# ramiyako/vector

Hardware: AMD Instinct MI355X
Metric: Msamples/s c64 through FIR+FFT+xcorr chain; 1/2/4/8 GPU + %HBM roofline (higher is better)
Workload: dtype c64 (fp32)

## Files before the change

vector_amd/csrc/refine.hip:

```cpp
#include "os_common.hpp"

namespace vsig {

#pragma clang fp contract(off)

template <class T> __device__ __forceinline__ double2 ld2(const T* p, long long i);
template <> __device__ __forceinline__ double2 ld2<float2>(const float2* p, long long i) {
  const float2 v = p[i];
  return make_double2((double)v.x, (double)v.y);
}
template <> __device__ __forceinline__ double2 ld2<double2>(const double2* p, long long i) {
  return p[i];
}
__device__ __forceinline__ double2 to_d2(float2 v) { return make_double2((double)v.x, (double)v.y); }
__device__ __forceinline__ double2 to_d2(double2 v) { return v; }

template <class U>
__device__ __forceinline__ void st_agent(U* p, U v) {
  __hip_atomic_store(p, v, __ATOMIC_RELAXED, __HIP_MEMORY_SCOPE_AGENT);
}
template <class U>
__device__ __forceinline__ U ld_agent(const U* p) {
  return __hip_atomic_load(p, __ATOMIC_RELAXED, __HIP_MEMORY_SCOPE_AGENT);
}
__device__ __forceinline__ void stores_done() { __builtin_amdgcn_s_waitcnt(0); }

__device__ __forceinline__ void tap_range(long long i, long long na, long long nv, long long& k0,
                                          long long& k1) {
  const long long lo = (nv - 1) - i;
  const long long hi = na + (nv - 1) - i;
  k0 = lo > 0 ? lo : 0;
  k1 = hi < nv ? hi : nv;
}


struct RefineSlot { double m; long long i; };

constexpr int kNpThreads = 256;
constexpr int kNpGrid = 512;
constexpr int kNpFast = 64;
constexpr int kTile = 2048;
constexpr int kTilePad = 8;
constexpr long long kBlasThreadMin = 10000;
constexpr long long kSparseMax = 4096;

struct RefineGeom {
  long long nout;
  long long F;
  long long na, nv;
  int rev;
  int from_array;
  long long hop;
  int waves, Q, stride;
  int wstep, rsub;
  int cols;
  int nthr;
  long long per_item;
  long long cap;
};

__device__ __forceinline__ long long row_offset(const RefineGeom& g, int w, int q, int l) {
  return (long long)g.wstep * w + l + 64LL * (q % g.rsub) + (long long)g.stride * (q / g.rsub);
}

__device__ __forceinline__ long long item_output(const RefineGeom& g, long long p, int q, int l) {
  const long long b = p / g.waves;
  const int w = (int)(p - b * g.waves);
  const long long ob = b * g.hop;
  const long long rem = g.nout - ob;
  const long long lim = rem < g.hop ? rem : g.hop;
  const long long r = row_offset(g, w, q, l);
  if (r >= lim) return -1;
  const long long raw = ob + r;
  return g.rev ? g.nout - 1 - raw : raw;
}

__device__ __forceinline__ long long entry_output(const RefineGeom& g, const long long* items,
                                                  long long e, long long it0 = -1,
                                                  long long item0 = 0) {
  const long long it = e / g.per_item;
  const int sub = (int)(e - it * g.per_item);
  const long long item = it == it0 ? item0 : ld_agent(items + it);
  if (g.from_array) {
    const long long raw = item * 64 + sub;
    return raw < g.nout ? raw : -1;
  }
  if (g.cols) return item_output(g, item >> 6, sub, (int)(item & 63));
  return item_output(g, item, sub >> 6, sub & 63);
}

__device__ __forceinline__ bool item_span(const RefineGeom& g, long long item, long long& lo,
                                          long long& hi) {
  long long rlo, rhi;
  if (g.from_array) {
    rlo = item * 64;
    if (rlo >= g.nout) return false;
    rhi = rlo + 63 < g.nout - 1 ? rlo + 63 : g.nout - 1;
    lo = rlo;
    hi = rhi;
    return true;
  }
  const long long p = g.cols ? item >> 6 : item;
  const int l = g.cols ? (int)(item & 63) : 0;
  const long long b = p / g.waves;
  const int w = (int)(p - b * g.waves);
  const long long ob = b * g.hop;
  const long long rem = g.nout - ob;
  const long long lim = rem < g.hop ? rem : g.hop;
  if (row_offset(g, w, 0, l) >= lim) return false;
  int qh = (g.cols ? g.cols : g.Q) - 1;
  while (row_offset(g, w, qh, l) >= lim) --qh;
  rlo = ob + row_offset(g, w, 0, l);
  long long top = row_offset(g, w, qh, l) + (g.cols ? 0 : 63);
  if (top >= lim) top = lim - 1;
  rhi = ob + top;
  if (g.rev) {
    lo = g.nout - 1 - rhi;
    hi = g.nout - 1 - rlo;
  } else {
    lo = rlo;
    hi = rhi;
  }
  return true;
}

__device__ __forceinline__ double band_threshold(const PeakPartial* rec, double eps) {
  const double t = rec->max2 * (1.0 - eps);
  return t > 0.0 ? t : 0.0;
}

__global__ __launch_bounds__(256) void refine_select_array(
    const float2* __restrict__ c, long long nout, const PeakPartial* __restrict__ rec, double eps,
    long long* __restrict__ items, RefineKeys* __restrict__ keys) {
  const long long i = (long long)blockIdx.x * 256 + threadIdx.x;
  const double t = band_threshold(rec, eps);
  const bool hit = i < nout && (double)hypotf(c[i].x, c[i].y) >= t;
  const unsigned long long m = __ballot(hit);
  if (hit && (threadIdx.x & 63) == (unsigned)__builtin_ctzll(m)) {
    const long long ch = i >> 6;
    const unsigned long long j = atomicAdd(&keys->count, 1ull);
    items[j] = ch;
    const long long hi = ch * 64 + 63 < nout - 1 ? ch * 64 + 63 : nout - 1;
    atomicMax(&keys->lo_inv, ~(unsigned long long)(ch * 64));
    atomicMax(&keys->hi_p1, (unsigned long long)(hi + 1));
  }
}
// ... 677 lines not shown
      else __builtin_amdgcn_s_sleep(127);
    }
    if (timed_out) watchdog_fired(f);
    skeys[0] = timed_out ? 0 : ld_agent(&f.keys->count);
    skeys[1] = ld_agent(&f.keys->lo_inv);
    skeys[2] = ld_agent(&f.keys->hi_p1);
    sitem0 = it0 < f.maxitems ? ld_agent(f.items + it0) : 0;
    stores_done();
    atomicAdd(&fc->seen, 1ull);
  }
  __syncthreads();
  long long nact;
  const bool last = numpy_pass<T>(a, v, f.g, f.items, f.keys, slots, cv, nullptr, 0, 0, f.rec,
                                  skeys[0], skeys[1], skeys[2], vb, kNpGrid, nact,
                                  (unsigned long long)it0 < skeys[0] ? it0 : -1, sitem0);
  if (tid == 0 && (last || (nact == 0 && vb == 0))) {
    const unsigned long long w0 = wall_clock64();
    while (__hip_atomic_load(&fc->seen, __ATOMIC_RELAXED, __HIP_MEMORY_SCOPE_AGENT) < (unsigned long long)kNpGrid) {
      if (wall_clock64() - w0 > f.wd_ticks) {
        watchdog_fired(f);
        break;
      }
      __builtin_amdgcn_s_sleep(20);
    }
    if (ld_agent(&f.keys->fault)) poison_record(f.rec);
    __hip_atomic_store(&fc->seen, 0ull, __ATOMIC_RELAXED, __HIP_MEMORY_SCOPE_AGENT);
    __hip_atomic_store(&fc->flag, 0ull, __ATOMIC_RELAXED, __HIP_MEMORY_SCOPE_AGENT);
    __hip_atomic_store(&fc->ticket, 0ull, __ATOMIC_RELAXED, __HIP_MEMORY_SCOPE_AGENT);
  }
}

static RefineGeom make_geom(const RefineArgs& r) {
  RefineGeom g{r.nout, r.F, r.na, r.nv, r.rev, r.from_array, r.hop, r.waves, r.Q, r.stride,
               r.wstep, r.rsub, r.cols, r.blas_threads > 1 ? r.blas_threads : 1, 0, r.cap};
  g.per_item = r.from_array ? 64 : r.cols ? r.cols : (long long)r.Q * 64;
  return g;
}

static long long max_items(const RefineArgs& r) {
  if (r.from_array) return (r.nout + 63) / 64;
  return r.cols ? r.nparts * 64 : r.nparts;
}

size_t refine_scratch_bytes(const RefineArgs& r) {
  return sizeof(RefineKeys) + (size_t)max_items(r) * 8 + kNpGrid * sizeof(RefineSlot);
}

static hipError_t launch_numpy(const RefineArgs& r, const RefineGeom& g, const long long* items,
                               RefineKeys* keys, RefineSlot* slots, double* vals, long long vlo,
                               long long vhi, hipStream_t st) {
  auto go = [&](auto tag) {
    using T = decltype(tag);
    hipLaunchKernelGGL(refine_numpy<T>, dim3(kNpGrid), dim3(kNpThreads), 0, st,
                       static_cast<const T*>(r.a), static_cast<const T*>(r.v), g, items, keys,
                       slots, static_cast<double2*>(r.out128), vals, vlo, vhi, r.rec);
  };
  if (r.c128) go(double2{});
  else go(float2{});
  return hipGetLastError();
}

hipError_t launch_refine(const RefineArgs& r, hipStream_t st) {
  if (r.cols && (r.from_array || r.cols > 64)) return hipErrorInvalidValue;
  char* base = static_cast<char*>(r.scratch);
  RefineKeys* keys = reinterpret_cast<RefineKeys*>(base);
  long long* items = reinterpret_cast<long long*>(base + sizeof(RefineKeys));
  RefineSlot* slots = reinterpret_cast<RefineSlot*>(items + max_items(r));
// ... 76 lines not shown
```

vector_amd/csrc/vsig_api.hip:

```cpp
#include <cmath>
#include <cstddef>
#include <cstdio>
#include <cstdlib>
#include <cstring>
#include <map>
#include <memory>
#include <string>
#include <vector>

#include "../../include/vsig.h"
#include "dtype.hpp"

using vsig::PeakPartial;
using vsig::dtype_bytes;
using vsig::dtype_ok;
static_assert(VSIG_DTYPE_C128 == vsig::VSIG_C128 && VSIG_DTYPE_C64 == vsig::VSIG_C64 &&
              VSIG_DTYPE_F64 == vsig::VSIG_F64 && VSIG_DTYPE_F32 == vsig::VSIG_F32, "VSIG_DTYPE_*");

struct TimingRec {
  std::vector<std::pair<hipEvent_t, hipEvent_t>> ev;
};

constexpr int kClockSlots = 32;

// ... 80 lines not shown
  int refine_async = 0;
  struct RefineAsync {
    hipStream_t stream = nullptr;
    hipEvent_t ev_corr = nullptr, ev_ref = nullptr;
    bool pending = false;
    bool joined = false;
    hipStream_t joined_on = nullptr;
  } ra;
  bool clock = false;
  DevBuf clkbuf;
  std::map<std::string, int> clkslot;
};

constexpr int kFirPartTaps = 8192;
struct vsig_fir {
  vsig_ctx* ctx;
  int ntaps, decim, M;
  long long hop;
  DevBuf Hs;
  DevBuf G;
  std::vector<vsig_fir*> parts;
  DevBuf z;
  ~vsig_fir() {
    (void)hipStreamSynchronize(ctx->stream);
    for (vsig_fir* p : parts) delete p;
  }
};

struct vsig_xcorr {
  vsig_ctx* ctx;
  long long L = 0;
  int M = 0;
  std::vector<DevBuf> Ps;
  DevBuf tmpl;
  DevBuf cbuf;
  explicit vsig_xcorr(vsig_ctx* c) : ctx(c) {}
  ~vsig_xcorr() { (void)hipStreamSynchronize(ctx->stream); }
};

constexpr long long kBankMaxL = 4096;
constexpr int kBankMaxK = 4096;
struct vsig_xcorr_bank {
  vsig_ctx* ctx;
  int K = 0;
  long long L = 0;
  int M = 0;
  DevBuf Ps;
  explicit vsig_xcorr_bank(vsig_ctx* c) : ctx(c) {}
  ~vsig_xcorr_bank() { (void)hipStreamSynchronize(ctx->stream); }
};

namespace {

int fail(vsig_ctx* c, int code, const std::string& msg) {
  if (c) c->err = msg;
  return code;
}

void join_refine(vsig_ctx* c) {
  vsig_ctx::RefineAsync& ra = c->ra;
  if (!ra.pending) return;
  if (ra.joined && ra.joined_on == c->stream) return;
  (void)hipStreamWaitEvent(c->stream, ra.ev_ref, 0);
  ra.joined = true;
  ra.joined_on = c->stream;
}
// ... 163 lines not shown

int clear_refine_fault(vsig_ctx* c, unsigned long long fault = 0) {
  char* keys = c->rscratch.as<char>();
  HIPCHK(c, hipMemsetAsync(keys, 0, sizeof(vsig::RefineKeys), c->stream));
  if (fault)
    HIPCHK(c, hipMemcpyAsync(keys + offsetof(vsig::RefineKeys, fault), &fault, sizeof(fault),
                             hipMemcpyHostToDevice, c->stream));
  if (c->parts())
    HIPCHK(c, hipMemsetAsync(c->counters(), 0, vsig::kCounterRecs * sizeof(PeakPartial), c->stream));
  HIPCHK(c, hipStreamSynchronize(c->stream));
  return VSIG_OK;
}

bool corr_span(int mode, long long na, long long nv, long long* F, long long* nout) {
  const long long nmin = na < nv ? na : nv, nmax = na < nv ? nv : na;
  if (mode == VSIG_MODE_FULL) { *F = 0; *nout = na + nv - 1; }
  else if (mode == VSIG_MODE_VALID) { *F = nmin - 1; *nout = nmax - nmin + 1; }
  else if (mode == VSIG_MODE_SAME) { *F = na >= nv ? nmin - 1 - nmin / 2 : nmin / 2; *nout = nmax; }
  else return false;
  return true;
}

bool is_complex_dtype(int dtype) { return dtype == VSIG_DTYPE_C64 || dtype == VSIG_DTYPE_C128; }

struct RefineOperands {
  const void* a; long long na;
  const void* v; long long nv;
  int c128;
  long long F;
};

int run_refine(vsig_ctx* c, const RefineOperands& op, long long nout, int M, long long hop,
               long long nparts, int rev, const float2* c64, PeakPartial* rec, void* out128,
               bool fused = false, const unsigned* lkeys = nullptr, bool async = false) {
  c->refine_ran = false;
  if (!c->refine) return fused ? fail(c, VSIG_E_INVALID, "refine: fused finalize with refine off")
                             : VSIG_OK;
  vsig::RefineArgs r{};
  r.a = op.a; r.na = op.na; r.v = op.v; r.nv = op.nv; r.c128 = op.c128;
  r.nout = nout; r.F = op.F; r.rev = rev;
  if (c64) {
    r.from_array = 1; r.c64 = c64; r.Q = 1; r.stride = 0; r.waves = 1; r.hop = 64;
    r.wstep = 64; r.rsub = 1;
  } else {
    int waves, Q, stride, plan, wstep, rsub;
    if (vsig::xcorr_geom(M, &waves, &Q, &stride, &plan, &wstep, &rsub) != hipSuccess)
      return fail(c, VSIG_E_INVALID, "refine: no correlator geometry for M");
    r.parts = c->parts(); r.nparts = nparts; r.hop = hop;
    r.waves = waves; r.Q = Q; r.stride = stride; r.wstep = wstep; r.rsub = rsub;
    if (fused) {
      r.finalize = 1;
      r.tmp = c->finalize_tmp();
      r.done = reinterpret_cast<unsigned long long*>(c->counters());
    }
    if (lkeys) {
      r.cols = Q; r.lkeys = lkeys; r.Q = 1;
    }
  }
  r.eps = c->refine_eps_ppm * 1e-6;
  r.blas_threads = c->blas_threads;
  r.cap = c->refine_cap;
  r.wd_ticks = (unsigned long long)c->refine_wd_us * 100ull;
  const size_t need = vsig::refine_scratch_bytes(r);
  const bool fresh = need > c->rscratch.bytes();
  unsigned long long pending_fault = 0;
  if (fresh && c->rscratch.data()) {
    vsig::RefineKeys keys;
    int rc = read_refine_keys(c, &keys);
    if (rc) return rc;
    pending_fault = keys.fault;
  }
  int rc = c->rscratch.reserve(c, need);
  if (rc) return rc;
  if (pending_fault) {
    if ((rc = clear_refine_fault(c, pending_fault))) return rc;
  } else if (fresh) {
    HIPCHK(c, hipMemsetAsync(c->rscratch.data(), 0, sizeof(vsig::RefineKeys), c->stream));
  }
  r.scratch = c->rscratch.data();
  r.rec = rec;
  r.out128 = out128;
  if (async && c->refine_async) {
// ... 682 lines not shown

int vsig_fir_c64(vsig_ctx* c, const void* x, int64_t n, const float* taps, int32_t ntaps,
                 int32_t decim, void* y, int64_t ny) {
  if (!c || !x || !taps || !y) return fail(c, VSIG_E_INVALID, "null pointer");
  if (ntaps < 1) return fail(c, VSIG_E_INVALID, "ntaps must be >= 1");
  std::vector<float2> tc(ntaps);
  for (int i = 0; i < ntaps; ++i) tc[i] = make_float2(taps[i], 0.f);
  vsig_fir* f = nullptr;
  int rc = vsig_fir_create(c, tc.data(), ntaps, decim, &f);
  if (rc) return rc;
  const std::unique_ptr<vsig_fir> owner(f);
  const size_t bx = (size_t)n * 8, by = (size_t)ny * 8;
  if ((rc = stage_in(c, 0, x, bx)) || (rc = c->stage[1].reserve(c, by)) ||
      (rc = vsig_fir_exec_dev(f, c->stage[0].data(), n, c->stage[1].data(), ny)) ||
      (rc = stage_out(c, y, c->stage[1], by)))
    return rc;
  HIPCHK(c, hipStreamSynchronize(c->stream));
  return VSIG_OK;
}

static int xcorr_build(vsig_ctx* c, const float2* td, long long L, vsig_xcorr* x) {
  constexpr long long B = 8192;
  x->L = L;
  x->M = os_size_xcorr(L) ? os_size_xcorr(L) : 16384;
  const long long Bc = x->M == 32768 ? 16384 : B;
  for (long long p = 0; p * Bc < L || p == 0; ++p) {
    const long long Lp = L <= Bc ? L : ((L - p * Bc) < B ? (L - p * Bc) : B);
    DevBuf P;
    const int rc = make_spectrum(c, td + p * B, (int)Lp, x->M, &P);
    if (rc) return rc;
    x->Ps.push_back(std::move(P));
    if (L <= Bc) break;
  }
  return VSIG_OK;
}

static int xcorr_run(vsig_xcorr* x, const float2* s, long long n, long long off, long long nout,
                     int store_mode, float2* cout, vsig_peak_t* peak_dev,
                     const RefineOperands* op, void* out128, bool async = false) {
  vsig_ctx* c = x->ctx;
  PeakPartial* rec = peak_record(c, peak_dev);
  if (x->Ps.size() == 1 && x->L <= (x->M == 32768 ? 16384 : 8192)) {
    long long hop = (long long)x->M - x->L + 1;
    if (x->M == 16384 && hop > 1) hop &= ~1LL;
    const long long nblocks = (nout + hop - 1) / hop;
    int waves, Q, stride, plan, wstep, rsub;
    if (vsig::xcorr_geom(x->M, &waves, &Q, &stride, &plan, &wstep, &rsub) != hipSuccess)
      return fail(c, VSIG_E_UNSUPPORTED, "correlator block size");
    const long long nparts = nblocks * waves;
    int rc = ensure_partials(c, nparts);
    if (rc) return rc;
    const bool fused = op && c->refine && !(store_mode & 8);
    unsigned* lk = nullptr;
    if (fused && Q <= 64 && vsig::xcorr_lane_keys(x->M) == Q) {
      if ((rc = c->lkeys.reserve(c, (size_t)nparts * 64 * sizeof(unsigned)))) return rc;
      lk = c->lkeys.as<unsigned>();
    }
    const float2* tw;
    const float2* wt = nullptr;
    if ((rc = get_twiddles(c, plan, &tw))) return rc;
    if (x->M >= 16384 && (rc = get_half_tw(c, x->M, x->M == 16384 ? 512 : 1024, &wt))) return rc;
    {
      Timed t(c, "xcorr");
      HIPCHK(c, vsig::launch_xcorr_os(x->M, s, n, x->Ps[0].as<float2>(), off, nout, hop, cout, store_mode,
                                      c->parts(), tw, wt, c->stream, lk));
    }
    if (!fused) {
      if ((rc = finalize_peak(c, nparts, 1, peak_dev))) return rc;
      if (!op) return VSIG_OK;
    }
    if (out128 && cout) HIPCHK(c, vsig::launch_convert_c(1, cout, nout, out128, c->stream));
    return run_refine(c, *op, nout, x->M, hop, nparts, (store_mode & 4) ? 1 : 0, nullptr, rec, out128,
                      fused, lk, async && peak_dev != nullptr);
  }
  constexpr long long B = 8192;
  constexpr int M = 16384;
  float2* cbuf = cout;
  int rc;
  if (!cbuf) {
    if ((rc = x->cbuf.reserve(c, (size_t)nout * sizeof(float2)))) return rc;
    cbuf = x->cbuf.as<float2>();
  }
  const float2 *tw, *wt;
  int waves, Q, stride, plan, wstep, rsub;
  if (vsig::xcorr_geom(M, &waves, &Q, &stride, &plan, &wstep, &rsub) != hipSuccess)
    return fail(c, VSIG_E_UNSUPPORTED, "correlator block size");
  if ((rc = get_twiddles(c, plan, &tw)) || (rc = get_half_tw(c, M, 512, &wt))) return rc;
  {
    Timed t(c, "xcorr");
    for (size_t p = 0; p < x->Ps.size(); ++p) {
      const long long Lp = (x->L - (long long)p * B) < B ? (x->L - (long long)p * B) : B;
      const int mode = (store_mode & 4 ? 2 | 4 : 1) | (p ? 8 : 0);
      HIPCHK(c, vsig::launch_xcorr_os(M, s, n, x->Ps[p].as<float2>(), off - (long long)p * B, nout,
                                      (long long)M - Lp + 1, cbuf, mode, nullptr, tw, wt,
                                      c->stream));
    }
    if ((rc = vsig_peak_dev(c, VSIG_DTYPE_C64, cbuf, nout, peak_dev))) return rc;
  }
  if (!op) return VSIG_OK;
  if (out128 && cout) HIPCHK(c, vsig::launch_convert_c(1, cout, nout, out128, c->stream));
  return run_refine(c, *op, nout, M, 0, 0, 0, cbuf, rec, out128);
}

int vsig_xcorr_create(vsig_ctx* c, const void* tmpl, int64_t L, vsig_xcorr** out) {
  if (!c || !tmpl || !out) return fail(c, VSIG_E_INVALID, "null pointer");
  *out = nullptr;
  if (L < 1) return fail(c, VSIG_E_INVALID, "template length must be >= 1");
  std::unique_ptr<vsig_xcorr> x(new vsig_xcorr(c));
  hipError_t e = x->tmpl.alloc((size_t)L * sizeof(float2));
  if (e == hipSuccess)
    e = hipMemcpyAsync(x->tmpl.data(), tmpl, (size_t)L * sizeof(float2), hipMemcpyHostToDevice, c->stream);
  if (e != hipSuccess)
    return fail(c, e == hipErrorOutOfMemory ? VSIG_E_NOMEM : VSIG_E_HIP, hipGetErrorString(e));
  const int rc = xcorr_build(c, x->tmpl.as<float2>(), L, x.get());
  (void)hipStreamSynchronize(c->stream);
  if (rc) return rc;
  *out = x.release();
  return VSIG_OK;
}

// ... 780 lines not shown
```

vector_amd/csrc/vsig_kernels.h:

```cpp
#pragma once
#include <hip/hip_runtime.h>

namespace vsig {

__device__ __forceinline__ long long xcd_remap(long long b, long long nb) {
  const long long q = nb >> 3, r = nb & 7;
  const long long x = b & 7, i = b >> 3;
  return x * q + (x < r ? x : r) + i;
}

struct ClockStamp {
  unsigned long long t0 = 0, r0 = 0;
  bool on;
  __device__ __forceinline__ ClockStamp(unsigned long long* sink, unsigned long long blk)
      : on(sink != nullptr && (blk & 63) == 0) {
    if (on) {
      t0 = __builtin_amdgcn_s_memtime();
      r0 = __builtin_amdgcn_s_memrealtime();
      __builtin_amdgcn_s_waitcnt(0xC07F);
    }
  }
  __device__ __forceinline__ void done(unsigned long long* sink) const {
    if (on && threadIdx.x < 2) {
      const unsigned long long t1 = __builtin_amdgcn_s_memtime();
// ... 54 lines not shown

hipError_t launch_psd(int N, const float2* x, long long stride, const float* win, int nperseg,
                      long long hop, float scale, float* out, long long nframes, int shift,
                      const float2* tw, hipStream_t st);
int psd_plan_threads(int N);
hipError_t launch_spectrum_prep(int N, const float2* u, int len, float gain, float2* S,
                                const float2* tw, hipStream_t st);
struct PsdRec { double sum; float mx, mn; };
struct PsdTracesPlan { long long blocks, step, fpb; };
constexpr int kPsdFoldRows = 8;
bool psd_traces_in_lds(long long N);
PsdTracesPlan psd_traces_plan(long long N, long long nframes);
int psd_traces_table(int N, bool* two_level);
hipError_t launch_psd_traces(int N, const float2* x, long long stride, const float* win, int nperseg,
                             long long hop, float scale, long long nframes, int shift, const float2* tw,
                             PsdRec* rows, hipStream_t st);
hipError_t launch_psd_traces_fold(const float* sxx, long long nb, long long N, int first, PsdRec* rows,
                                  hipStream_t st);
hipError_t launch_psd_traces_merge(const PsdRec* rows, long long nrows, long long N, long long nframes,
                                   double* mean, float* mx, float* mn, hipStream_t st);
hipError_t launch_fir_dec(int decim, const float2* x, long long n, long long g0, const float2* Hs,
                          int lo2, long long hop, float2* y, const float2* tw, const float2* twd,
                          hipStream_t st, const MixArgs* mix = nullptr);
hipError_t launch_fir_poly_gtable(const float2* Hs, float2* G, hipStream_t st);
hipError_t launch_fir_poly(const float2* x, long long n, long long g0, const float2* G, int lo2,
                           long long hop, float2* y, const float2* tw, const float2* twd,
                           hipStream_t st, const MixArgs* mix = nullptr);
hipError_t launch_fir_os(int M, const float2* x, long long n, long long g0, const float2* Hs,
                         int ntaps, long long hop, int decim, float2* y, const float2* tw,
                         hipStream_t st, const MixArgs* mix = nullptr);
hipError_t launch_xcorr_os(int M, const float2* s, long long n, const float2* Ps, long long off,
                           long long nout, long long hop, float2* c, int store_mode,
                           PeakPartial* partials, const float2* tw, const float2* wt,
                           hipStream_t st, unsigned* lkeys = nullptr);
int xcorr_lane_keys(int M);
hipError_t xcorr_geom(int M, int* waves, int* Q, int* stride, int* plan, int* wstep, int* rsub);
hipError_t xcorr_bank_geom(int M, long long nblocks, int* waves, long long* grid);
hipError_t launch_xcorr_bank(int M, const float2* s, long long n, const float2* Ps, int K,
                             long long off, long long nout, long long hop, float2* c,
                             PeakPartial* partials, const float2* tw, hipStream_t st);
hipError_t launch_bank_finalize(const PeakPartial* parts, int K, long long nparts, PeakPartial* out,
                                hipStream_t st);
#ifdef VSIG_TUNING
hipError_t launch_fft_bench(int key, float2* io, int frames, int iters, const float2* tw, int twl,
                            hipStream_t st);
hipError_t launch_copy_probe(const float2* x, long long n, float2* y, int variant, int grid,
                             hipStream_t st);
#endif
hipError_t launch_peak_reduce(int dtype, const void* a, long long n, PeakPartial* partials,
                              int nparts, hipStream_t st);
hipError_t launch_peak_first_nan(int dtype, const void* a, long long n, PeakPartial* rec, hipStream_t st);
constexpr int kFinalizeTmp = 1024;
constexpr int kCounterRecs = 4;
hipError_t launch_partial_finalize(const PeakPartial* parts, long long nparts, int sqrt_max,
                                   PeakPartial* out, PeakPartial* tmp, hipStream_t st);

struct RefineArgs {
  const void* a; long long na;
  const void* v; long long nv;
  int c128;
  long long nout, F;
  int rev;
  int from_array;
  const float2* c64;
  const PeakPartial* parts;
  long long nparts, hop;
  int waves, Q, stride;
  int wstep, rsub;
  double eps;
  int blas_threads;
  int cols;
  const unsigned* lkeys;
  int finalize;
  PeakPartial* tmp;
  unsigned long long* done;
  long long cap;
  void* scratch;
  PeakPartial* rec;
  void* out128;
  unsigned long long wd_ticks;
};
struct RefineKeys {
  unsigned long long count;
  unsigned long long lo_inv;
  unsigned long long hi_p1;
  unsigned long long status;
  unsigned long long done;
  unsigned long long fault;
  unsigned long long pad[2];
};
constexpr size_t kRefineKeysBytes = 64;
static_assert(sizeof(RefineKeys) == kRefineKeysBytes, "the items follow the keys at +64 B");
size_t refine_scratch_bytes(const RefineArgs& r);
hipError_t launch_refine(const RefineArgs& r, hipStream_t st);
size_t refine_values_scratch_bytes();
hipError_t launch_refine_values(const RefineArgs& r, long long lo, long long hi, double* vals,
                                hipStream_t st);
size_t np_stats_scratch_bytes(long long n);
hipError_t launch_np_stats(int dtype, const void* a, long long n, double* out, void* scratch,
                           hipStream_t st);
constexpr int kRegionBlocks = 2048;
// ... 119 lines not shown
```

vector_amd/csrc/xcorr.hip:

```cpp
#include "xcorr_epilogue.hpp"

namespace vsig {

template <class P>
__global__ __launch_bounds__(P::TF) void xcorr_os_kernel(
    const float2* __restrict__ s, long long n, const float2* __restrict__ Ps, long long off,
    long long nout, long long hop, float2* __restrict__ c, int store_mode,
    PeakPartial* __restrict__ partials, long long nblocks, const float2* __restrict__ tw) {
  static_assert(P::R[0] == P::RL, "overlap-save needs a palindromic plan");
  __shared__ __attribute__((aligned(16))) float2 lds[lds_size<P>()];
  const int t = threadIdx.x;
  long long b = blockIdx.x;
  if (b >= nblocks) return;
  float2 wa[nanch_total<P>()];
  load_anchors<P>(wa, tw, t);
  float2 v[P::E];
  load_segment<P>(v, s, b * hop - off, n, t);
  for (; b < nblocks; b += gridDim.x) {
    fft_frame_anch<P>(v, lds, wa, t);
#pragma unroll
    for (int e = 0; e < P::E; ++e) v[e] = cmul(cconj(v[e]), Ps[out_index<P>(t, e)]);
    float2 nv[P::E];
    const long long nb = b + gridDim.x;
    if (nb < nblocks) load_segment<P>(nv, s, nb * hop - off, n, t);
// ... 5 lines not shown
}

using PlanX32k = Plan16384w;
using PlanX16k = Plan8192c;
constexpr int kPlanKey16k = -8192;

template <class P, int M>
constexpr int half_root(int e) {
  return ((e / P::R[0]) * P::TF + (e % P::R[0]) * (P::N / P::R[0])) / (M / 64);
}

template <class P>
__device__ __forceinline__ void load_halves(float2* a, float2* d, const float2* __restrict__ x,
                                            long long s0, long long n, int t) {
  constexpr int H = P::N;
  const float2* base = x + s0;
  if (s0 >= 0 && s0 + 2 * H <= n) {
    const auto rs = make_rsrc(base, 2u * H * (unsigned)sizeof(float2));
    const unsigned v0 = (unsigned)in_index<P>(t, 0) * (unsigned)sizeof(float2);
    static_for<0, P::E>([&](auto ei) {
      constexpr int e = decltype(ei)::value;
      a[e] = buf_load2(rs, v0, in_off<P>(e) * (int)sizeof(float2));
      d[e] = buf_load2(rs, v0, (in_off<P>(e) + H) * (int)sizeof(float2));
    });
  } else {
#pragma unroll
    for (int e = 0; e < P::E; ++e) {
      const int i = in_index<P>(t, e);
      const long long x0 = s0 + i, x1 = x0 + H;
      a[e] = (x0 >= 0 && x0 < n) ? base[i] : make_float2(0.f, 0.f);
      d[e] = (x1 >= 0 && x1 < n) ? base[i + H] : make_float2(0.f, 0.f);
    }
  }
}

template <class P>
struct KeyedRank {
  static constexpr int c(int e) { return (e / P::RL) * P::TF + (e % P::RL) * (P::N / P::RL); }
  static constexpr int rank(int e) {
    int r = 0;
    for (int q = 0; q < P::E; ++q) r += c(q) < c(e);
    return r;
  }
  static constexpr int kStep = P::TF < P::N / P::RL ? P::TF : P::N / P::RL;
  static constexpr bool check() {
    if (mapl_of<P>::value == kMapIlv || 2 * P::E > 64 || P::N != kStep * P::E) return false;
    for (int e = 0; e < P::E; ++e)
      if (c(e) != kStep * rank(e)) return false;
    return true;
  }
  static constexpr bool ok = check();
};

template <class P, int DV = -1>
__device__ __forceinline__ void xcorr_half_epilogue(const float2* a, const float2* d, long long b,
                                                    long long hop, long long nout,
                                                    float2* __restrict__ c, int store_mode,
                                                    PeakPartial* partials, unsigned* lkeys, int t) {
  constexpr int H = P::N;
  const long long ob = b * hop;
  const long long rem = nout - ob;
  const int lim = rem < hop ? (int)rem : (int)hop;
  const bool rev = store_mode & 4;
  const bool accum = store_mode & 8;
  const int smode = store_mode & 3;
  if (smode == 1) {
// ... 77 lines not shown
    return;
  }
  float m = -1.f, s1 = 0.f, s2 = 0.f;
  int mi = 0;
  auto acc = [&](float2 v, int i) {
    const bool ok = i < lim;
    const float a2r = v.x * v.x + v.y * v.y;
    const float a2 = ok ? a2r : -1.f;
    const bool take = (a2 > m) | (rev & (a2 == m) & ok);
    m = take ? a2 : m;
    mi = take ? i : mi;
    s1 += ok ? __builtin_amdgcn_sqrtf(a2r) : 0.f;
    s2 += ok ? a2r : 0.f;
  };
  if (!rev && lim > H) {
#pragma unroll
    for (int e = 0; e < P::E; ++e) {
      const float a2 = a[e].x * a[e].x + a[e].y * a[e].y;
      const bool take = a2 > m;
      m = take ? a2 : m;
      mi = take ? out_index<P>(t, e) : mi;
      s1 += __builtin_amdgcn_sqrtf(a2);
      s2 += a2;
    }
  } else {
#pragma unroll
    for (int e = 0; e < P::E; ++e) acc(a[e], out_index<P>(t, e));
  }
#pragma unroll
  for (int e = 0; e < P::E; ++e) acc(d[e], out_index<P>(t, e) + H);
  wave_partial_f(m, mi, s1, s2, rev, ob, nout, partials + b * (P::TF / 64) + (t >> 6));
}

template <class P>
constexpr int xcorr_waves_per_eu() { return P::E <= 16 ? 4 : P::TF >= 512 ? 1 : 2; }

constexpr int kSegPfDist = 64;

template <class P, int DV = -1>
__global__ __launch_bounds__(P::TF, xcorr_waves_per_eu<P>()) void xcorr_half_kernel(
    const float2* __restrict__ s, long long n, const float4* __restrict__ Ps2, long long off,
    long long nout, long long hop, float2* __restrict__ c, int store_mode,
    PeakPartial* __restrict__ partials, long long nblocks, const float2* __restrict__ tw,
    const float2* __restrict__ wt, unsigned* __restrict__ lkeys, unsigned long long* clk) {
  static_assert(P::R[0] == P::RL, "overlap-save needs a palindromic plan");
  static_assert(map0_of<P>::value != kMapIlv, "one split twiddle per thread");
  constexpr int M = 2 * P::N;
  static_assert(P::TF % (M / 64) == 0 && (P::N / P::R[0]) % (M / 64) == 0,
                "per-element split twiddles must be 64th roots of unity");
  __shared__ __attribute__((aligned(16))) float2 lds[lds_size<P>()];
  const int t = threadIdx.x;
  const ClockStamp cs(clk, blockIdx.x);
  float2 wa[nanch_total<P>()];
  load_anchors<P>(wa, tw, t);
  float2 wx[twx_total<P>()];
  load_twx<P>(wx, tw, t);
  const long long b = xcd_remap(blockIdx.x, gridDim.x);
  if (b >= nblocks) return;
  auto fft2 = [&](float2* x, float2* y) {
    launder_anchors<P>(wa);
    fft_pair<P>(x, y, lds, TwAnchorsX{wa, wx}, t);
  };
  const float2 w = wt[in_index<P>(t, 0)];
  float2 a[P::E], d[P::E];
  load_halves<P>(a, d, s, b * hop - off, n, t);
  constexpr int kPfLines = 2 * P::N * 8 / 128 / P::TF;
  float pfv[kPfLines];
#pragma unroll
  for (int k = 0; k < kPfLines; ++k) pfv[k] = 0.f;
  static_for<0, P::E>([&](auto ei) {
    constexpr int e = decltype(ei)::value;
    const float2 x0 = a[e], x1 = d[e];
    a[e] = cadd(x0, x1);
    d[e] = twc<half_root<P, M>(e), 64>(cmul(csub(x0, x1), w));
  });
  fft2(a, d);
  {
    const auto rp = make_rsrc(Ps2, (unsigned)P::N * (unsigned)sizeof(float4));
    const unsigned v0 = (unsigned)out_index<P>(t, 0) * (unsigned)sizeof(float4);
    static_for<0, P::E>([&](auto ei) {
      constexpr int e = decltype(ei)::value;
      const float4 p = buf_load4(rp, v0, out_off<P>(e) * (int)sizeof(float4));
      a[e] = cmul(cconj(a[e]), make_float2(p.x, p.y));
      d[e] = cmul(cconj(d[e]), make_float2(p.z, p.w));
    });
  }
  fft2(a, d);
  static_for<0, P::E>([&](auto ei) {
    constexpr int e = decltype(ei)::value;
    const float2 o = twc<half_root<P, M>(e), 64>(cmul(d[e], w));
    const float2 ev = a[e];
    a[e] = cadd(ev, o);
    d[e] = csub(ev, o);
  });
  {
    const long long bn = b + kSegPfDist;
    const long long s0 = bn * hop - off;
    if (bn < nblocks && s0 >= 0 && s0 + 2 * P::N <= n) {
      const float* q = reinterpret_cast<const float*>(s + s0);
#pragma unroll
      for (int k = 0; k < kPfLines; ++k) pfv[k] = q[(t + k * P::TF) * 32];
    }
  }
  xcorr_half_epilogue<P, DV>(a, d, b, hop, nout, c, store_mode, partials, lkeys, t);
#pragma unroll
  for (int k = 0; k < kPfLines; ++k)
    asm volatile("" ::"v"(pfv[k]));
  cs.done(clk);
}

hipError_t launch_xcorr_os(int M, const float2* s, long long n, const float2* Ps, long long off,
                           long long nout, long long hop, float2* c, int store_mode,
                           PeakPartial* partials, const float2* tw, const float2* wt,
                           hipStream_t st, unsigned* lkeys) {
  if (nout <= 0) return hipSuccess;
  if (lkeys && !xcorr_lane_keys(M)) return hipErrorInvalidValue;
  const long long nblocks = (nout + hop - 1) / hop;
  if (M == 16384) {
    using KR = KeyedRank<PlanX16k>;
    constexpr int kDv = PlanX16k::E / 2;
    const long long cut = hop - PlanX16k::N;
    const bool dv = KR::ok && KR::kStep == PlanX16k::TF && cut == (long long)kDv * KR::kStep;
    if (dv) {
      hipLaunchKernelGGL((xcorr_half_kernel<PlanX16k, kDv>), dim3((unsigned)nblocks),
                         dim3(PlanX16k::TF), 0, st, s, n, reinterpret_cast<const float4*>(Ps), off, nout,
                         hop, c, store_mode, partials, nblocks, tw, wt, lkeys, g_clock_sink);
      return hipGetLastError();
    }
    hipLaunchKernelGGL(xcorr_half_kernel<PlanX16k>, dim3((unsigned)nblocks), dim3(PlanX16k::TF), 0,
                       st, s, n, reinterpret_cast<const float4*>(Ps), off, nout, hop, c, store_mode,
                       partials, nblocks, tw, wt, lkeys, g_clock_sink);
    return hipGetLastError();
  }
  if (M == 32768) {
    hipLaunchKernelGGL(xcorr_half_kernel<PlanX32k>, dim3((unsigned)nblocks), dim3(PlanX32k::TF), 0,
                       st, s, n, reinterpret_cast<const float4*>(Ps), off, nout, hop, c, store_mode,
                       partials, nblocks, tw, wt, lkeys, g_clock_sink);
    return hipGetLastError();
  }
  auto run = [&](auto plan) {
    using PL = decltype(plan);
    auto k = xcorr_os_kernel<PL>;
    const long long grid = persistent_grid(k, PL::TF, nblocks);
    hipLaunchKernelGGL(k, dim3((unsigned)grid), dim3(PL::TF), 0, st, s, n, Ps, off, nout, hop, c,
                       store_mode, partials, nblocks, tw);
  };
  if (M == 4096) run(Plan4096{});
  else if (M == 8192) run(Plan8192{});
  else return hipErrorInvalidValue;
  return hipGetLastError();
}

template <class P>
constexpr int lane_key_rows() {
  return KeyedRank<P>::ok && KeyedRank<P>::kStep == P::TF && 2 * P::E <= 64 ? 2 * P::E : 0;
}
int xcorr_lane_keys(int M) {
  if (M == 16384) return lane_key_rows<PlanX16k>();
  if (M == 32768) return lane_key_rows<PlanX32k>();
  return 0;
}

hipError_t xcorr_geom(int M, int* waves, int* Q, int* stride, int* plan, int* wstep, int* rsub) {
  *wstep = 64;
  *rsub = 1;
  if (M == 32768) { *waves = PlanX32k::TF / 64; *Q = 2 * PlanX32k::E; *stride = PlanX32k::TF; *plan = -16384; }
  else if (M == 16384) {
    *waves = PlanX16k::TF / 64; *Q = 2 * PlanX16k::E; *stride = PlanX16k::TF; *plan = kPlanKey16k;
  }
  else if (M == 8192) { *waves = Plan8192::TF / 64; *Q = Plan8192::E; *stride = Plan8192::TF; *plan = 8192; }
  else if (M == 4096) { *waves = Plan4096::TF / 64; *Q = Plan4096::E; *stride = Plan4096::TF; *plan = 4096; }
  else return hipErrorInvalidValue;
  return hipSuccess;
}

}
```

Measured before the change: 313,600.

## Add even/odd parity-split path for the 16k half-size correlator

Adds a parity variant of the M=16384 half-length correlator. It loads even/odd samples as one float4 and uses a precomputed sum/difference spectrum table (SD) with a folded twiddle. This removes the pre-FFT and post-FFT butterfly/twiddle passes, moving that work into the pointwise multiply with fused complex MACs. Output indexing, peak keys and refine geometry get new lane/row steps so the interleaved layout still maps to the right output positions. The path runs only when the input pointer and offset are parity-aligned, and it costs an extra table buffer plus a new kernel variant.

After: 319,500, median of 6. 1.02x the previous value.

```diff
diff --git a/vector_amd/csrc/refine.hip b/vector_amd/csrc/refine.hip
--- a/vector_amd/csrc/refine.hip
+++ b/vector_amd/csrc/refine.hip
@@ -53,6 +53,7 @@
   long long hop;
   int waves, Q, stride;
   int wstep, rsub;
+  int lstep, rstep;
   int cols;
   int nthr;
   long long per_item;
@@ -60,7 +61,8 @@
 };
 
 __device__ __forceinline__ long long row_offset(const RefineGeom& g, int w, int q, int l) {
-  return (long long)g.wstep * w + l + 64LL * (q % g.rsub) + (long long)g.stride * (q / g.rsub);
+  return (long long)g.wstep * w + (long long)g.lstep * l + (long long)g.rstep * (q % g.rsub) +
+         (long long)g.stride * (q / g.rsub);
 }
 
 __device__ __forceinline__ long long item_output(const RefineGeom& g, long long p, int q, int l) {
@@ -111,7 +113,7 @@
   int qh = (g.cols ? g.cols : g.Q) - 1;
   while (row_offset(g, w, qh, l) >= lim) --qh;
   rlo = ob + row_offset(g, w, 0, l);
-  long long top = row_offset(g, w, qh, l) + (g.cols ? 0 : 63);
+  long long top = g.cols ? row_offset(g, w, qh, l) : row_offset(g, w, qh, 63);
   if (top >= lim) top = lim - 1;
   rhi = ob + top;
   if (g.rev) {
@@ -855,7 +857,8 @@
 
 static RefineGeom make_geom(const RefineArgs& r) {
   RefineGeom g{r.nout, r.F, r.na, r.nv, r.rev, r.from_array, r.hop, r.waves, r.Q, r.stride,
-               r.wstep, r.rsub, r.cols, r.blas_threads > 1 ? r.blas_threads : 1, 0, r.cap};
+               r.wstep, r.rsub, r.lstep ? r.lstep : 1, r.rstep ? r.rstep : 64, r.cols,
+               r.blas_threads > 1 ? r.blas_threads : 1, 0, r.cap};
   g.per_item = r.from_array ? 64 : r.cols ? r.cols : (long long)r.Q * 64;
   return g;
 }
diff --git a/vector_amd/csrc/vsig_api.hip b/vector_amd/csrc/vsig_api.hip
--- a/vector_amd/csrc/vsig_api.hip
+++ b/vector_amd/csrc/vsig_api.hip
@@ -136,6 +136,7 @@
   long long L = 0;
   int M = 0;
   std::vector<DevBuf> Ps;
+  DevBuf SD;
   DevBuf tmpl;
   DevBuf cbuf;
   explicit vsig_xcorr(vsig_ctx* c) : ctx(c) {}
@@ -365,7 +366,8 @@
 
 int run_refine(vsig_ctx* c, const RefineOperands& op, long long nout, int M, long long hop,
                long long nparts, int rev, const float2* c64, PeakPartial* rec, void* out128,
-               bool fused = false, const unsigned* lkeys = nullptr, bool async = false) {
+               bool fused = false, const unsigned* lkeys = nullptr, bool async = false,
+               bool parity = false) {
   c->refine_ran = false;
   if (!c->refine) return fused ? fail(c, VSIG_E_INVALID, "refine: fused finalize with refine off")
                              : VSIG_OK;
@@ -376,11 +378,13 @@
     r.from_array = 1; r.c64 = c64; r.Q = 1; r.stride = 0; r.waves = 1; r.hop = 64;
     r.wstep = 64; r.rsub = 1;
   } else {
-    int waves, Q, stride, plan, wstep, rsub;
-    if (vsig::xcorr_geom(M, &waves, &Q, &stride, &plan, &wstep, &rsub) != hipSuccess)
+    vsig::XcorrGeom g;
+    if (vsig::xcorr_geom(M, parity, &g) != hipSuccess)
       return fail(c, VSIG_E_INVALID, "refine: no correlator geometry for M");
+    const int Q = g.Q;
     r.parts = c->parts(); r.nparts = nparts; r.hop = hop;
-    r.waves = waves; r.Q = Q; r.stride = stride; r.wstep = wstep; r.rsub = rsub;
+    r.waves = g.waves; r.Q = g.Q; r.stride = g.stride; r.wstep = g.wstep; r.rsub = g.rsub;
+    r.lstep = g.lstep; r.rstep = g.rstep;
     if (fused) {
       r.finalize = 1;
       r.tmp = c->finalize_tmp();
@@ -1129,6 +1133,10 @@
     x->Ps.push_back(std::move(P));
     if (L <= Bc) break;
   }
+  if (x->M == 16384 && x->Ps.size() == 1) {
+    HIPCHK(c, x->SD.alloc((size_t)(x->M / 2) * sizeof(float4)));
+    HIPCHK(c, vsig::launch_xcorr_parity_table(x->M, x->Ps[0].as<float2>(), x->SD.as<float4>(), c->stream));
+  }
   return VSIG_OK;
 }
 
@@ -1141,9 +1149,11 @@
     long long hop = (long long)x->M - x->L + 1;
     if (x->M == 16384 && hop > 1) hop &= ~1LL;
     const long long nblocks = (nout + hop - 1) / hop;
-    int waves, Q, stride, plan, wstep, rsub;
-    if (vsig::xcorr_geom(x->M, &waves, &Q, &stride, &plan, &wstep, &rsub) != hipSuccess)
+    const bool parity = x->M == 16384 && x->SD.data() && !(hop & 1) && vsig::xcorr_parity_aligned(s, off);
+    vsig::XcorrGeom g;
+    if (vsig::xcorr_geom(x->M, parity, &g) != hipSuccess)
       return fail(c, VSIG_E_UNSUPPORTED, "correlator block size");
+    const int waves = g.waves, Q = g.Q, plan = g.plan;
     const long long nparts = nblocks * waves;
     int rc = ensure_partials(c, nparts);
     if (rc) return rc;
@@ -1160,7 +1170,8 @@
     {
       Timed t(c, "xcorr");
       HIPCHK(c, vsig::launch_xcorr_os(x->M, s, n, x->Ps[0].as<float2>(), off, nout, hop, cout, store_mode,
-                                      c->parts(), tw, wt, c->stream, lk));
+                                      c->parts(), tw, wt, c->stream, lk,
+                                      parity ? x->SD.as<float4>() : nullptr));
     }
     if (!fused) {
       if ((rc = finalize_peak(c, nparts, 1, peak_dev))) return rc;
@@ -1168,7 +1179,7 @@
     }
     if (out128 && cout) HIPCHK(c, vsig::launch_convert_c(1, cout, nout, out128, c->stream));
     return run_refine(c, *op, nout, x->M, hop, nparts, (store_mode & 4) ? 1 : 0, nullptr, rec, out128,
-                      fused, lk, async && peak_dev != nullptr);
+                      fused, lk, async && peak_dev != nullptr, parity);
   }
   constexpr long long B = 8192;
   constexpr int M = 16384;
@@ -1179,10 +1190,10 @@
     cbuf = x->cbuf.as<float2>();
   }
   const float2 *tw, *wt;
-  int waves, Q, stride, plan, wstep, rsub;
-  if (vsig::xcorr_geom(M, &waves, &Q, &stride, &plan, &wstep, &rsub) != hipSuccess)
+  vsig::XcorrGeom g;
+  if (vsig::xcorr_geom(M, false, &g) != hipSuccess)
     return fail(c, VSIG_E_UNSUPPORTED, "correlator block size");
-  if ((rc = get_twiddles(c, plan, &tw)) || (rc = get_half_tw(c, M, 512, &wt))) return rc;
+  if ((rc = get_twiddles(c, g.plan, &tw)) || (rc = get_half_tw(c, M, 512, &wt))) return rc;
   {
     Timed t(c, "xcorr");
     for (size_t p = 0; p < x->Ps.size(); ++p) {
diff --git a/vector_amd/csrc/vsig_kernels.h b/vector_amd/csrc/vsig_kernels.h
--- a/vector_amd/csrc/vsig_kernels.h
+++ b/vector_amd/csrc/vsig_kernels.h
@@ -110,9 +110,12 @@
 hipError_t launch_xcorr_os(int M, const float2* s, long long n, const float2* Ps, long long off,
                            long long nout, long long hop, float2* c, int store_mode,
                            PeakPartial* partials, const float2* tw, const float2* wt,
-                           hipStream_t st, unsigned* lkeys = nullptr);
+                           hipStream_t st, unsigned* lkeys = nullptr, const float4* SD = nullptr);
+hipError_t launch_xcorr_parity_table(int M, const float2* Ps, float4* SD, hipStream_t st);
+bool xcorr_parity_aligned(const float2* s, long long off);
 int xcorr_lane_keys(int M);
-hipError_t xcorr_geom(int M, int* waves, int* Q, int* stride, int* plan, int* wstep, int* rsub);
+struct XcorrGeom { int waves, Q, stride, plan, wstep, rsub, lstep, rstep; };
+hipError_t xcorr_geom(int M, bool parity, XcorrGeom* g);
 hipError_t xcorr_bank_geom(int M, long long nblocks, int* waves, long long* grid);
 hipError_t launch_xcorr_bank(int M, const float2* s, long long n, const float2* Ps, int K,
                              long long off, long long nout, long long hop, float2* c,
@@ -145,6 +148,7 @@
   long long nparts, hop;
   int waves, Q, stride;
   int wstep, rsub;
+  int lstep, rstep;
   double eps;
   int blas_threads;
   int cols;
diff --git a/vector_amd/csrc/xcorr.hip b/vector_amd/csrc/xcorr.hip
--- a/vector_amd/csrc/xcorr.hip
+++ b/vector_amd/csrc/xcorr.hip
@@ -61,6 +61,47 @@
       d[e] = (x1 >= 0 && x1 < n) ? base[i + H] : make_float2(0.f, 0.f);
     }
   }
+}
+
+template <class P>
+__device__ __forceinline__ void load_parity(float2* a, float2* d, const float2* __restrict__ x,
+                                            long long s0, long long n, int t) {
+  constexpr int H = P::N;
+  const float2* base = x + s0;
+  if (s0 >= 0 && s0 + 2 * H <= n) {
+    const auto rs = make_rsrc(base, 2u * H * (unsigned)sizeof(float2));
+    const unsigned v0 = (unsigned)in_index<P>(t, 0) * (unsigned)sizeof(float4);
+    static_for<0, P::E>([&](auto ei) {
+      constexpr int e = decltype(ei)::value;
+      const float4 q = buf_load4(rs, v0, in_off<P>(e) * (int)sizeof(float4));
+      a[e] = make_float2(q.x, q.y);
+      d[e] = make_float2(q.z, q.w);
+    });
+  } else {
+#pragma unroll
+    for (int e = 0; e < P::E; ++e) {
+      const int i = 2 * in_index<P>(t, e);
+      const long long x0 = s0 + i, x1 = x0 + 1;
+      a[e] = (x0 >= 0 && x0 < n) ? base[i] : make_float2(0.f, 0.f);
+      d[e] = (x1 >= 0 && x1 < n) ? base[i + 1] : make_float2(0.f, 0.f);
+    }
+  }
+}
+
+template <class P>
+constexpr int parity_root(int e) { return out_off<P>(e) / (P::N / 64); }
+
+__device__ __forceinline__ float2 cmac(float2 a, float2 b, float2 acc) {
+  const f2v av = tov(a), bv = tov(b);
+  return cmul_fin(a, b, av * bv.xx + tov(acc));
+}
+__device__ __forceinline__ float2 cmsub(float2 a, float2 b, float2 acc) {
+  const f2v av = tov(a), bv = tov(b);
+  const f2v t = tov(acc) - av * bv.xx;
+  f2v r;
+  asm("v_pk_fma_f32 %0, %1, %2, %3 op_sel:[1,1,0] op_sel_hi:[0,1,1] neg_hi:[1,0,0]"
+      : "=v"(r) : "v"(av), "v"(bv), "v"(t));
+  return fromv(r);
 }
 
 template <class P>
@@ -204,12 +245,96 @@
   wave_partial_f(m, mi, s1, s2, rev, ob, nout, partials + b * (P::TF / 64) + (t >> 6));
 }
 
+template <class P, int DV = -1>
+__device__ __forceinline__ void xcorr_parity_epilogue(const float2* a, const float2* d,
+                                                      long long b, long long hop, long long nout,
+                                                      float2* __restrict__ c, int store_mode,
+                                                      PeakPartial* partials, unsigned* lkeys,
+                                                      int t) {
+  using KR = KeyedRank<P>;
+  static_assert(KR::ok && KR::kStep == P::TF, "the parity split keys by 2 rank + parity");
+  const long long ob = b * hop;
+  const long long rem = nout - ob;
+  const int lim = rem < hop ? (int)rem : (int)hop;
+  const bool rev = store_mode & 4;
+  const bool accum = store_mode & 8;
+  const int smode = store_mode & 3;
+  if (smode == 1) {
+#pragma unroll
+    for (int e = 0; e < P::E; ++e) {
+      const int i = 2 * out_index<P>(t, e);
+      if (i < lim) put_c(c + ob + (unsigned)i, cconj(a[e]), accum);
+      if (i + 1 < lim) put_c(c + ob + (unsigned)(i + 1), cconj(d[e]), accum);
+    }
+  } else if (smode == 2) {
+#pragma unroll
+    for (int e = 0; e < P::E; ++e) {
+      const int i = 2 * out_index<P>(t, e);
+      if (i < lim) put_c(c + (nout - 1 - ob) - i, a[e], accum);
+      if (i + 1 < lim) put_c(c + (nout - 1 - ob) - (i + 1), d[e], accum);
+    }
+  }
+  if (!partials) return;
+  auto keyed = [&](auto revc) {
+    constexpr bool kRev = decltype(revc)::value;
+    constexpr unsigned rx = kRev ? 0u : 63u;
+    unsigned key = 0u;
+    bool any = false;
+    float s1 = 0.f, s2 = 0.f;
+    auto acc = [&](float2 v, int i, int k6, auto masked) {
+      const float a2 = v.x * v.x + v.y * v.y;
+      const unsigned k = (__float_as_uint(a2) & ~63u) | ((unsigned)k6 ^ rx);
+      if constexpr (decltype(masked)::value) {
+        const bool ok = i < lim;
+        key = ok ? (k > key ? k : key) : key;
+        any |= ok;
+        s1 += ok ? __builtin_amdgcn_sqrtf(a2) : 0.f;
+        s2 += ok ? a2 : 0.f;
+      } else {
+        key = k > key ? k : key;
+        any = true;
+        s1 += __builtin_amdgcn_sqrtf(a2);
+        s2 += a2;
+      }
+    };
+    if (DV >= 0 && lim == hop) {
+      static_for<0, P::E>([&](auto ei) {
+        constexpr int e = decltype(ei)::value;
+        if constexpr (KR::rank(e) < DV) {
+          acc(a[e], 0, 2 * KR::rank(e), IC<0>{});
+          acc(d[e], 0, 2 * KR::rank(e) + 1, IC<0>{});
+        }
+      });
+    } else {
+      static_for<0, P::E>([&](auto ei) {
+        constexpr int e = decltype(ei)::value;
+        constexpr int c0 = 2 * KR::kStep * KR::rank(e);
+        if (c0 + 2 * KR::kStep <= lim) {
+          acc(a[e], 0, 2 * KR::rank(e), IC<0>{});
+          acc(d[e], 0, 2 * KR::rank(e) + 1, IC<0>{});
+        } else if (c0 < lim) {
+          const int i = 2 * out_index<P>(t, e);
+          acc(a[e], i, 2 * KR::rank(e), IC<1>{});
+          acc(d[e], i + 1, 2 * KR::rank(e) + 1, IC<1>{});
+        }
+      });
+    }
+    if (lkeys) lkeys[b * P::TF + tmapl<P>(t)] = key;
+    const int k6 = (int)((key & 63u) ^ rx);
+    const int mi = 2 * (tmapl<P>(t) + KR::kStep * (k6 >> 1)) + (k6 & 1);
+    const float m = any ? __uint_as_float(key & ~63u) : -1.f;
+    wave_partial_f(m, mi, s1, s2, kRev, ob, nout, partials + b * (P::TF / 64) + (t >> 6));
+  };
+  if (rev) keyed(IC<1>{});
+  else keyed(IC<0>{});
+}
+
 template <class P>
 constexpr int xcorr_waves_per_eu() { return P::E <= 16 ? 4 : P::TF >= 512 ? 1 : 2; }
 
 constexpr int kSegPfDist = 64;
 
-template <class P, int DV = -1>
+template <class P, int DV = -1, bool PS = false>
 __global__ __launch_bounds__(P::TF, xcorr_waves_per_eu<P>()) void xcorr_half_kernel(
     const float2* __restrict__ s, long long n, const float4* __restrict__ Ps2, long long off,
     long long nout, long long hop, float2* __restrict__ c, int store_mode,
@@ -233,19 +358,22 @@
     launder_anchors<P>(wa);
     fft_pair<P>(x, y, lds, TwAnchorsX{wa, wx}, t);
   };
-  const float2 w = wt[in_index<P>(t, 0)];
+  const float2 w = wt[PS ? 2 * out_index<P>(t, 0) : in_index<P>(t, 0)];
   float2 a[P::E], d[P::E];
-  load_halves<P>(a, d, s, b * hop - off, n, t);
+  if constexpr (PS) load_parity<P>(a, d, s, b * hop - off, n, t);
+  else load_halves<P>(a, d, s, b * hop - off, n, t);
   constexpr int kPfLines = 2 * P::N * 8 / 128 / P::TF;
   float pfv[kPfLines];
 #pragma unroll
   for (int k = 0; k < kPfLines; ++k) pfv[k] = 0.f;
-  static_for<0, P::E>([&](auto ei) {
-    constexpr int e = decltype(ei)::value;
-    const float2 x0 = a[e], x1 = d[e];
-    a[e] = cadd(x0, x1);
-    d[e] = twc<half_root<P, M>(e), 64>(cmul(csub(x0, x1), w));
-  });
+  if constexpr (!PS) {
+    static_for<0, P::E>([&](auto ei) {
+      constexpr int e = decltype(ei)::value;
+      const float2 x0 = a[e], x1 = d[e];
+      a[e] = cadd(x0, x1);
+      d[e] = twc<half_root<P, M>(e), 64>(cmul(csub(x0, x1), w));
+    });
+  }
   fft2(a, d);
   {
     const auto rp = make_rsrc(Ps2, (unsigned)P::N * (unsigned)sizeof(float4));
@@ -253,18 +381,30 @@
     static_for<0, P::E>([&](auto ei) {
       constexpr int e = decltype(ei)::value;
       const float4 p = buf_load4(rp, v0, out_off<P>(e) * (int)sizeof(float4));
-      a[e] = cmul(cconj(a[e]), make_float2(p.x, p.y));
-      d[e] = cmul(cconj(d[e]), make_float2(p.z, p.w));
+      if constexpr (PS) {
+        const float2 S = make_float2(p.x, p.y), D = make_float2(p.z, p.w);
+        constexpr int K = parity_root<P>(e);
+        const float2 Dw = twc<K % 32, 64>(cmul(D, w));
+        const float2 ce = cconj(a[e]), co = cconj(d[e]);
+        a[e] = cmac(co, D, cmul(ce, S));
+        if constexpr (K < 32) d[e] = cmac(ce, Dw, cmul(co, S));
+        else d[e] = cmsub(ce, Dw, cmul(co, S));
+      } else {
+        a[e] = cmul(cconj(a[e]), make_float2(p.x, p.y));
+        d[e] = cmul(cconj(d[e]), make_float2(p.z, p.w));
+      }
     });
   }
   fft2(a, d);
-  static_for<0, P::E>([&](auto ei) {
-    constexpr int e = decltype(ei)::value;
-    const float2 o = twc<half_root<P, M>(e), 64>(cmul(d[e], w));
-    const float2 ev = a[e];
-    a[e] = cadd(ev, o);
-    d[e] = csub(ev, o);
-  });
+  if constexpr (!PS) {
+    static_for<0, P::E>([&](auto ei) {
+      constexpr int e = decltype(ei)::value;
+      const float2 o = twc<half_root<P, M>(e), 64>(cmul(d[e], w));
+      const float2 ev = a[e];
+      a[e] = cadd(ev, o);
+      d[e] = csub(ev, o);
+    });
+  }
   {
     const long long bn = b + kSegPfDist;
     const long long s0 = bn * hop - off;
@@ -274,34 +414,64 @@
       for (int k = 0; k < kPfLines; ++k) pfv[k] = q[(t + k * P::TF) * 32];
     }
   }
-  xcorr_half_epilogue<P, DV>(a, d, b, hop, nout, c, store_mode, partials, lkeys, t);
+  if constexpr (PS) xcorr_parity_epilogue<P, DV>(a, d, b, hop, nout, c, store_mode, partials, lkeys, t);
+  else xcorr_half_epilogue<P, DV>(a, d, b, hop, nout, c, store_mode, partials, lkeys, t);
 #pragma unroll
   for (int k = 0; k < kPfLines; ++k)
     asm volatile("" ::"v"(pfv[k]));
   cs.done(clk);
 }
 
+__global__ __launch_bounds__(256) void xcorr_parity_table_kernel(const float2* __restrict__ P,
+                                                                 float4* __restrict__ SD, int H) {
+  const int k = blockIdx.x * 256 + threadIdx.x;
+  if (k >= H) return;
+  const float2 p0 = P[k], p1 = P[k + H];
+  const double dr = (double)p0.x - (double)p1.x, di = (double)p0.y - (double)p1.y;
+  double sn, cs;
+  sincospi((double)k / (double)H, &sn, &cs);
+  SD[k] = make_float4((float)((double)p0.x + (double)p1.x), (float)((double)p0.y + (double)p1.y),
+                      (float)(dr * cs - di * sn), (float)(dr * sn + di * cs));
+}
+
+hipError_t launch_xcorr_parity_table(int M, const float2* Ps, float4* SD, hipStream_t st) {
+  if (M != 16384) return hipErrorInvalidValue;
+  const int H = M / 2;
+  hipLaunchKernelGGL(xcorr_parity_table_kernel, dim3((H + 255) / 256), dim3(256), 0, st, Ps, SD, H);
+  return hipGetLastError();
+}
+
+bool xcorr_parity_aligned(const float2* s, long long off) {
+  return (((long long)(reinterpret_cast<unsigned long long>(s) >> 3) - off) & 1) == 0;
+}
+
 hipError_t launch_xcorr_os(int M, const float2* s, long long n, const float2* Ps, long long off,
                            long long nout, long long hop, float2* c, int store_mode,
                            PeakPartial* partials, const float2* tw, const float2* wt,
-                           hipStream_t st, unsigned* lkeys) {
+                           hipStream_t st, unsigned* lkeys, const float4* SD) {
   if (nout <= 0) return hipSuccess;
   if (lkeys && !xcorr_lane_keys(M)) return hipErrorInvalidValue;
+  if (SD && (M != 16384 || (hop & 1) || (reinterpret_cast<unsigned long long>(s) & 7) ||
+             !xcorr_parity_aligned(s, off)))
+    return hipErrorInvalidValue;
   const long long nblocks = (nout + hop - 1) / hop;
   if (M == 16384) {
     using KR = KeyedRank<PlanX16k>;
     constexpr int kDv = PlanX16k::E / 2;
+    constexpr int kDvPs = (PlanX16k::N + kDv * KR::kStep) / (2 * KR::kStep);
     const long long cut = hop - PlanX16k::N;
     const bool dv = KR::ok && KR::kStep == PlanX16k::TF && cut == (long long)kDv * KR::kStep;
-    if (dv) {
-      hipLaunchKernelGGL((xcorr_half_kernel<PlanX16k, kDv>), dim3((unsigned)nblocks),
-                         dim3(PlanX16k::TF), 0, st, s, n, reinterpret_cast<const float4*>(Ps), off, nout,
-                         hop, c, store_mode, partials, nblocks, tw, wt, lkeys, g_clock_sink);
-      return hipGetLastError();
-    }
-    hipLaunchKernelGGL(xcorr_half_kernel<PlanX16k>, dim3((unsigned)nblocks), dim3(PlanX16k::TF), 0,
-                       st, s, n, reinterpret_cast<const float4*>(Ps), off, nout, hop, c, store_mode,
-                       partials, nblocks, tw, wt, lkeys, g_clock_sink);
+    auto run = [&](auto kern, const float4* tab) {
+      hipLaunchKernelGGL(kern, dim3((unsigned)nblocks), dim3(PlanX16k::TF), 0, st, s, n, tab, off,
+                         nout, hop, c, store_mode, partials, nblocks, tw, wt, lkeys, g_clock_sink);
+    };
+    if (SD) {
+      if (dv) run(xcorr_half_kernel<PlanX16k, kDvPs, true>, SD);
+      else run(xcorr_half_kernel<PlanX16k, -1, true>, SD);
+    } else {
+      if (dv) run(xcorr_half_kernel<PlanX16k, kDv>, reinterpret_cast<const float4*>(Ps));
+      else run(xcorr_half_kernel<PlanX16k>, reinterpret_cast<const float4*>(Ps));
+    }
     return hipGetLastError();
   }
   if (M == 32768) {
@@ -333,15 +503,16 @@
   return 0;
 }
 
-hipError_t xcorr_geom(int M, int* waves, int* Q, int* stride, int* plan, int* wstep, int* rsub) {
-  *wstep = 64;
-  *rsub = 1;
-  if (M == 32768) { *waves = PlanX32k::TF / 64; *Q = 2 * PlanX32k::E; *stride = PlanX32k::TF; *plan = -16384; }
+hipError_t xcorr_geom(int M, bool parity, XcorrGeom* g) {
+  g->wstep = 64; g->rsub = 1; g->lstep = 1; g->rstep = 64;
+  if (parity && M != 16384) return hipErrorInvalidValue;
+  if (M == 32768) { g->waves = PlanX32k::TF / 64; g->Q = 2 * PlanX32k::E; g->stride = PlanX32k::TF; g->plan = -16384; }
   else if (M == 16384) {
-    *waves = PlanX16k::TF / 64; *Q = 2 * PlanX16k::E; *stride = PlanX16k::TF; *plan = kPlanKey16k;
-  }
-  else if (M == 8192) { *waves = Plan8192::TF / 64; *Q = Plan8192::E; *stride = Plan8192::TF; *plan = 8192; }
-  else if (M == 4096) { *waves = Plan4096::TF / 64; *Q = Plan4096::E; *stride = Plan4096::TF; *plan = 4096; }
+    g->waves = PlanX16k::TF / 64; g->Q = 2 * PlanX16k::E; g->stride = PlanX16k::TF; g->plan = kPlanKey16k;
+    if (parity) { g->wstep = 128; g->lstep = 2; g->rsub = 2; g->rstep = 1; g->stride = 2 * PlanX16k::TF; }
+  }
+  else if (M == 8192) { g->waves = Plan8192::TF / 64; g->Q = Plan8192::E; g->stride = Plan8192::TF; g->plan = 8192; }
+  else if (M == 4096) { g->waves = Plan4096::TF / 64; g->Q = Plan4096::E; g->stride = Plan4096::TF; g->plan = 4096; }
   else return hipErrorInvalidValue;
   return hipSuccess;
 }
```
